# terasum/mythril

Hardware: AMD Instinct MI355X
Metric: constraint-evals/sec (higher is better)
Workload: dtype u32; 1 GPU; synthetic config 5: 10000 random 256-bit constraint tapes x 67108864 assignments per GPU, throughput mode; variant=plain, tapes=10000, rows_per_gpu=67108864, rows_total=67108864, vars=4, mode=count_all, engine=jit, short_circuit=True, parallelism=dp1 (row shards, all-reduce of per-tape results)

## Files before the change

### mythril_amd/csrc/jit.cpp

```cpp
#include "jit.h"

#include <stdarg.h>
#include <stdio.h>
#include <string.h>

#include <algorithm>
#include <atomic>
#include <climits>
#include <cstdlib>
#include <stdexcept>
#include <string>
#include <thread>
#include <unordered_map>
#include <vector>

namespace mh {
namespace jit {

namespace {

struct Fail {
    std::string why;
};

[[noreturn]] void fail(const std::string& w) { throw Fail{w}; }

enum LK : uint8_t { L_UNDEF, L_CONST, L_VGPR };
struct Limb {
    uint8_t k = L_UNDEF;
    uint32_t v = 0;
    static Limb C(uint32_t x) { Limb l; l.k = L_CONST; l.v = x; return l; }
    static Limb R(uint32_t r) { Limb l; l.k = L_VGPR; l.v = r; return l; }
    bool is_c() const { return k == L_CONST; }
    bool is_r() const { return k == L_VGPR; }
    bool is_c(uint32_t x) const { return k == L_CONST && v == x; }
};

struct Val {
    bool is_bool = false;
    int bconst = -1;
    int pair = -1;
    Limb l[8];
    bool defined = false;
};

enum : uint32_t { LBL_SC_SKIP = 0xFFF0, LBL_SC_END = 0xFFF1 };

int top_bit(uint32_t m) { return m ? 31 - __builtin_clz(m) : -1; }
uint32_t prefix_mask(uint32_t m) { int t = top_bit(m); return t < 0 ? 0u : ((2u << t) - 1u); }

class Emitter {
public:
    Emitter(const SsaTape& st, const std::vector<uint32_t>& pool, uint32_t n_vars,
            const Options& opt, const std::vector<uint8_t>* check = nullptr,
            std::vector<double>* insn_cost = nullptr)
        : st_(st), pool_(pool), n_vars_(n_vars), opt_(opt), check_(check),
          insn_cost_(insn_cost) {}

    TapeCode run();

private:
    const SsaTape& st_;
    const std::vector<uint32_t>& pool_;
    uint32_t n_vars_;
    Options opt_;
    const std::vector<uint8_t>* check_;
    std::vector<double>* insn_cost_;
    bool sc_used_ = false;
    std::vector<MI> code_;
    std::vector<Val> vals_;
    std::vector<int> last_;
    std::vector<uint8_t> dem_;
    int vref_[512] = {};
    uint32_t vbase_ = 0, vmax_ = 0, vhigh_ = 0;
    int pref_[N_BOOL_PAIRS] = {};
    uint32_t kstage_ = 0;
    uint32_t n_valu_ = 0, n_wide_ = 0, n_salu_ = 0;
    uint32_t n_valu_cold_ = 0;
    int cold_ = 0;
    bool calls_div_ = false;
    bool uses_lds_ = false;
    bool calls_kec_ = false;
    int cur_op_ = -1;
public:
    static uint64_t op_valu[256], op_wide[256], op_count[256];
// ... 146 lines not shown
    int chain(bool sub, const Limb* a, const Limb* b, int top, Limb* res, uint32_t junk,
              std::vector<uint32_t>& tmp);
    void op_addsub(int d, const Val& A, const Val& B, bool sub);
    void op_logic(int d, const Val& A, const Val& B, int kind);
    Val op_eq(const Val& A, const Val& B);
    void and_all_zero(const std::vector<uint32_t>& regs, int* p, std::vector<uint32_t>& tmp);
    Val op_ult(const Val& A, const Val& B, bool signed_, bool negate);
    void op_ite(int d, const Val& C, const Val& T, const Val& E);
    Val op_bite(const Val& C, const Val& T, const Val& E);
    Val op_bool2(uint8_t op, const Val& A, const Val& B);
    void op_shr(int d, const Val& A, uint32_t s);
    void op_shl(int d, const Val& A, uint32_t s);
    void op_vshift(int d, const Val& A, const Val& B, uint8_t op);
    void op_mul(int d, const Val& A, const Val& B);
    void op_div(int d, int a, int b, int cidx, uint32_t kind, int cur);
    void rescue_div_regs(int cur, uint32_t end = R_TEMP0);
    void op_keccak(const SsaInsn& v, int cur);
    void op_exp(int d, const Val& A, const Val& E);
    void addmod_regs(const uint32_t* u, const uint32_t* v, const uint32_t* n, uint32_t* r,
                     int when = -1);
    void op_mulmod(int d, const Val& X, const Val& Y, const Val& N);
    int scratch_ = -1;
    void demand();
    void sc_check(const Val& v);
    Val& out(int d) {
        Val& v = vals_[d];
        v = Val();
        v.defined = true;
        return v;
    }
};

int Emitter::chain(bool sub, const Limb* a, const Limb* b, int top, Limb* res, uint32_t junk,
                   std::vector<uint32_t>& tmp) {
    int cs = 0;
    uint32_t same = ~0u;
    for (int k = 0; k <= top; ++k) {
        const Limb x = a[k], y = b[k];
        if (x.k == L_UNDEF || y.k == L_UNDEF) fail("internal: chain over an undemanded limb");
        if (cs == 2 && x.is_c() && y.is_c()) {
            const bool through = sub ? x.v == y.v : (uint64_t)x.v + y.v == 0xFFFFFFFFull;
            if (through) {
                if (res) {
                    if (same == ~0u) {
                        same = valloc();
                        emit(M_V_ADDC_CO, {V(same), S(S_DIV_DUMMY, 2), IMM(sub ? 0u : ~0u),
                                           IMM(sub ? 0u : 0u), VCC()}, true);
// ... 76 lines not shown
                    const uint32_t qr = vgpr_of(q, tmp);
                    emit(M_V_ADDC_CO, {V(dst), VCC(), vi_of(p, tmp), V(qr), VCC()});
                }
            } else {
                if (y.is_r()) {
                    emit(M_V_SUBB_CO, {V(dst), VCC(), vi_of(x, tmp), V(y.v), VCC()});
                } else if (x.is_r()) {
                    emit(M_V_SUBBREV_CO, {V(dst), VCC(), vi_of(y, tmp), V(x.v), VCC()});
                } else if (is_inline(x.v) && is_inline(y.v)) {
                    emit(M_V_SUBB_CO, {V(dst), VCC(), IMM(x.v), IMM(y.v), VCC()}, true);
                } else {
                    emit(M_V_SUBB_CO, {V(dst), VCC(), vi_of(x, tmp), V(vgpr_of(y, tmp)), VCC()});
                }
            }
        }
        cs = 2;
        if (res) res[k] = Limb::R(dst);
    }
    return cs;
}

void Emitter::op_addsub(int d, const Val& A, const Val& B, bool sub) {
    const int top = top_bit(dem_[d]);
    Val& R = out(d);
    if (top < 0) return;
    std::vector<uint32_t> tmp;
    chain(sub, A.l, B.l, top, R.l, 0, tmp);
    free_tmp(tmp);
}

void Emitter::op_logic(int d, const Val& A, const Val& B, int kind) {
    const uint32_t dm = dem_[d];
    Val& R = out(d);
    for (int k = 0; k < 8; ++k) {
        if (!((dm >> k) & 1)) continue;
        Limb x = A.l[k], y = B.l[k];
        if (x.is_c() && !y.is_c()) std::swap(x, y);
        if (y.is_c() && ((kind == 0 && y.v == 0) || (kind == 1 && y.v == ~0u))) {
            R.l[k] = Limb::C(y.v);
            continue;
        }
        if (x.k == L_UNDEF || y.k == L_UNDEF) fail("internal: logic over an undemanded limb");
        auto alias = [&](const Limb& l) { R.l[k] = l; if (l.is_r()) vretain(l.v); };
        if (x.is_c() && y.is_c()) {
            R.l[k] = Limb::C(kind == 0 ? (x.v & y.v) : kind == 1 ? (x.v | y.v) : (x.v ^ y.v));
            continue;
// ... 849 lines not shown
                if (l.is_c()) emit(M_V_MOV, {V(dst), IMM(__builtin_bswap32(l.v))});
                else emit(M_V_PERM, {V(dst), IMM(0), V(l.v), S(S_PERM_SEL)});
            }
    free_tmp(tmp);
    for (uint32_t lane = 4 * nw; lane < 25; ++lane)
        for (uint32_t h = 0; h < 2; ++h) {
            uint32_t x = 0;
            if (full && lane == 4 * nw && h == 0) x = 1u;
            if (lane == 16 && h == 1) x = 0x80000000u;
            emit(M_V_MOV, {V(R_KEC0 + 2 * lane + h), IMM(x)});
        }
    emit(M_CALL_KEC, {IMM((uint32_t)code_.size())});
    const KecCode& kc = kec_routine();
    Val& R = out(v.d);
    const uint32_t dm = dem_[v.d];
    for (int k = 0; k < 8; ++k) {
        if (!((dm >> k) & 1)) continue;
        const uint32_t r = valloc();
        emit(M_V_PERM, {V(r), IMM(0), V(kc.out[7 - k]), S(S_PERM_SEL)});
        R.l[k] = Limb::R(r);
    }
}

void Emitter::demand() {
    const auto& code = st_.code;
    const int nv = st_.n_vregs;
    dem_.assign(nv, 0);
    if (st_.root >= 0) dem_[st_.root] = 0xFF;
    auto D = [&](int r, uint32_t m) { if (r >= 0) dem_[r] |= (uint8_t)m; };
    for (size_t i = code.size(); i-- > 0;) {
        const SsaInsn& v = code[i];
        const uint32_t dd = dem_[v.d];
        const uint8_t op = v.op;
        switch (op) {
            case D_NOP: D(v.a, dd); break;
            case D_ADD_R: case D_SUB_R: case D_RSUB_R: case D_MUL_R:
                D(v.a, prefix_mask(dd));
                D(v.b, prefix_mask(dd));
                break;
            case D_AND_R: case D_OR_R: case D_XOR_R: {
                uint32_t ma = dd;
                if (v.cidx >= 0) {
                    for (int k = 0; k < 8; ++k) {
                        const uint32_t c = pool_[8ull * (uint32_t)v.cidx + k];
                        if ((op == D_AND_R && c == 0) || (op == D_OR_R && c == ~0u))
                            ma &= ~(1u << k);
                    }
                }
                D(v.a, ma);
                D(v.b, dd);
                break;
            }
            case D_ITE: D(v.b, dd); D(v.c, dd); break;
            case D_EXP: case D_MULMOD:
                D(v.a, 0xFF);
                D(v.b, 0xFF);
                D(v.c, 0xFF);
                break;
            case D_SHL_V: case D_LSHR_V: case D_ASHR_V:
                D(v.a, 0xFF);
                D(v.b, 0xFF);
                break;
            default:
                if (op >= D_SHR0 && op <= D_SHR7) {
                    const uint32_t s = 32u * (op - D_SHR0) + (v.aux & 31u);
                    const uint32_t q = s >> 5, bsh = s & 31;
                    uint32_t m = 0;
                    for (int k = 0; k < 8; ++k)
                        if ((dd >> k) & 1) {
                            if (k + q < 8) m |= 1u << (k + q);
                            if (bsh && k + q + 1 < 8) m |= 1u << (k + q + 1);
                        }
                    D(v.a, m);
                } else if (op >= D_SHL0 && op <= D_SHL7) {
                    const uint32_t p = op - D_SHL0, f = v.aux & 31u;
                    const uint32_t s = f ? 32u * p + 32u - f : 32u * (p + 1u);
                    if (s < 256) {
                        const int q = (int)(s >> 5), bsh = (int)(s & 31);
                        uint32_t m = 0;
                        for (int k = 0; k < 8; ++k)
                            if ((dd >> k) & 1) {
                                if (k - q >= 0) m |= 1u << (k - q);
                                if (bsh && k - q - 1 >= 0) m |= 1u << (k - q - 1);
                            }
                        D(v.a, m);
                    }
                } else if ((op >= D_EQ_R && op <= D_SGE_C) ||
                           (op >= D_UDIV_R && op <= D_SMOD_C)) {
                    D(v.a, 0xFF);
                    D(v.b, 0xFF);
                } else if (op == D_KECCAK) {
                    D(v.a, 0xFF);
                    D(v.b, 0xFF);
                    D(v.c, 0xFF);
                } else {
                    D(v.a, 0);
                }
                break;
        }
    }
}

uint64_t Emitter::op_valu[256], Emitter::op_wide[256], Emitter::op_count[256];

void Emitter::sc_check(const Val& v) {
    if (!v.is_bool || v.bconst == 1) return;
    sc_used_ = true;
    if (v.bconst == 0) {
        emit(M_S_BRANCH, {LBL(LBL_SC_SKIP)});
        return;
    }
    emit(M_S_AND_B64, {S(S_SCRATCH, 2), P(v.pair), S(S_VALID, 2)});
    emit(M_S_CBRANCH_SCC0, {LBL(LBL_SC_SKIP)});
}

namespace {

double sc_cost(const SsaInsn& v) {
    const uint8_t op = v.op;
    if (op == D_MUL_R) return 60;
    if (op >= D_UDIV_R && op <= D_SMOD_C) return 130;
    if (op == D_SHL_V || op == D_LSHR_V || op == D_ASHR_V) return 35;
    if (op == D_KECCAK) return 7000;
// ... 179 lines not shown
        const int k = order[s];
        for (int i : cone[k])
            if (!done[i]) { out.code.push_back(code[i]); done[i] = 1; }
        if (acc < 0) {
            acc = conj[k];
            check[acc] = 1;
            continue;
        }
        SsaInsn a{};
        a.op = D_BAND;
        a.d = s + 1 == order.size() ? st.root : chain_d[next_d++];
        a.a = acc;
        a.b = conj[k];
        a.c = -1;
        a.width = 1;
        a.cidx = -1;
        out.code.push_back(a);
        acc = a.d;
        if (acc != st.root) check[acc] = 1;
    }
    return true;
}

TapeCode Emitter::run() {
    TapeCode tc;
    tc.alg_ops = st_.alg_ops;
    try {
        const auto& code = st_.code;
        const int nv = st_.n_vregs;
        if (insn_cost_) insn_cost_->assign(code.size(), 0.0);
        const uint32_t n_pin = pinned_cols(n_vars_);
        if (st_.n_pinned != (int)n_pin) fail("assignment columns not pinned as the module pins them");
        bool has_div = false, has_kec = false;
        for (const SsaInsn& v : code) {
            if (v.op == D_KECCAK) { has_kec = true; continue; }
            if (v.op == D_LOADVAR || v.op == D_EXP) continue;
            if (v.op == D_MULMOD && (v.aux & 2u)) continue;
            if (v.op >= D_FIRST_COMPLEX) {
                fail(v.op == D_EXP ? "EXP with a symbolic exponent (interpreter only)"
                     : v.op == D_MULMOD ? "MULMOD (interpreter only)"
                                        : "complex op (interpreter only)");
            }
            if (v.op >= D_UDIV_R && v.op <= D_SMOD_C) has_div = true;
        }
        vbase_ = has_kec ? R_TEMP_KEC : has_div ? R_TEMP0 : n_pin ? R_TEMP_NODIV : R_COL0;
        vmax_ = std::min<uint32_t>(has_kec ? std::max(opt_.max_vgpr, opt_.max_vgpr_keccak)
                                           : opt_.max_vgpr, 256);
        if (vmax_ <= vbase_ + 16) fail("VGPR budget too small");
        vhigh_ = R_COL0 + 8 * n_pin;
        vals_.assign(nv, Val());
        for (int c = 0; c < st_.n_pinned; ++c) {
            Val& v = vals_[c];
            v.defined = true;
            for (int k = 0; k < 8; ++k) v.l[k] = Limb::R(R_COL0 + 8u * (uint32_t)c + k);
        }
        last_.assign(nv, -1);
        for (int i = 0; i < (int)code.size(); ++i)
            for (int r : {code[i].a, code[i].b, code[i].c})
                if (r >= 0) last_[r] = i;
        if (st_.root >= 0) last_[st_.root] = INT_MAX;
        demand();
        scratch_ = nv;
        vals_.push_back(Val());
        last_.push_back(-1);
        dem_.push_back(0xFF);
        for (int i = 0; i < (int)code.size(); ++i) {
            const SsaInsn& v = code[i];
            const uint8_t op = v.op;
            cur_op_ = op;
            const uint32_t valu_before = n_valu_, cold_before = n_valu_cold_;
            ++op_count[op];
            auto Y = [&]() -> Val { return v.cidx >= 0 ? const_val(v.cidx) : val(v.b); };
            switch (op) {
                case D_NOP: {
                    const Val& a = val(v.a);
                    retain(a);
                    vals_[v.d] = a;
                    break;
                }
                case D_LOADC: vals_[v.d] = const_val(v.cidx); break;
                case D_LOADVAR: {
                    const uint32_t dm = dem_[v.d];
                    Val& R = out(v.d);
                    for (int k = 0; k < 8; ++k)
                        if ((dm >> k) & 1u) {
                            const uint32_t r = valloc();
                            emit(M_LOADCOL, {V(r), IMM(8u * v.aux + (uint32_t)k)});
                            R.l[k] = Limb::R(r);
                        }
                    if (dm) emit(M_S_WAITCNT_VM, {IMM(0)});
                    break;
                }
                case D_TRUE: vals_[v.d] = bool_const(true); break;
                case D_FALSE: vals_[v.d] = bool_const(false); break;
                case D_ADD_R: op_addsub(v.d, val(v.a), Y(), false); break;
                case D_SUB_R: op_addsub(v.d, val(v.a), Y(), true); break;
                case D_RSUB_R: op_addsub(v.d, Y(), val(v.a), true); break;
                case D_AND_R: op_logic(v.d, val(v.a), Y(), 0); break;
                case D_OR_R: op_logic(v.d, val(v.a), Y(), 1); break;
                case D_XOR_R: op_logic(v.d, val(v.a), Y(), 2); break;
                case D_EQ_R: vals_[v.d] = op_eq(val(v.a), Y()); break;
                case D_ULT_R: vals_[v.d] = op_ult(val(v.a), Y(), false, false); break;
                case D_UGE_R: vals_[v.d] = op_ult(val(v.a), Y(), false, true); break;
                case D_UGT_R: vals_[v.d] = op_ult(Y(), val(v.a), false, false); break;
                case D_ULE_R: vals_[v.d] = op_ult(Y(), val(v.a), false, true); break;
                case D_SLT_R: vals_[v.d] = op_ult(val(v.a), Y(), true, false); break;
                case D_SGE_R: vals_[v.d] = op_ult(val(v.a), Y(), true, true); break;
                case D_SGT_R: vals_[v.d] = op_ult(Y(), val(v.a), true, false); break;
                case D_SLE_R: vals_[v.d] = op_ult(Y(), val(v.a), true, true); break;
                case D_BAND: case D_BOR: case D_BXOR: case D_BEQ:
                    vals_[v.d] = op_bool2(op, val(v.a), val(v.b));
                    break;
                case D_BNOT: {
                    const Val& a = val(v.a);
                    if (a.bconst >= 0) {
                        vals_[v.d] = bool_const(!a.bconst);
                    } else {
                        const int p = palloc();
                        emit(M_S_NOT_B64, {P(p), P(a.pair)});
                        vals_[v.d] = bool_mask(p);
                    }
                    break;
                }
                case D_ITE: op_ite(v.d, val(v.a), val(v.b), val(v.c)); break;
                case D_BITE: vals_[v.d] = op_bite(val(v.a), val(v.b), val(v.c)); break;
                case D_MUL_R: op_mul(v.d, val(v.a), Y()); break;
                case D_SHL_V: case D_LSHR_V: case D_ASHR_V:
                    op_vshift(v.d, val(v.a), val(v.b), op);
                    break;
                case D_UDIV_R: case D_UREM_R: case D_SDIV_R: case D_SREM_R: case D_SMOD_R:
                    op_div(v.d, v.a, v.b, v.cidx, (uint32_t)(op - D_UDIV_R) >> 1, i);
                    break;
                case D_KECCAK: op_keccak(v, i); break;
                case D_EXP: op_exp(v.d, val(v.a), Y()); break;
                case D_MULMOD: op_mulmod(v.d, val(v.a), val(v.b), val(v.c)); break;
                default:
                    if (op >= D_SHR0 && op <= D_SHR7) {
                        const uint32_t s = 32u * (op - D_SHR0) + (v.aux & 31u);
                        if (s == 0) { const Val& a = val(v.a); retain(a); vals_[v.d] = a; }
                        else op_shr(v.d, val(v.a), s);
                    } else if (op >= D_SHL0 && op <= D_SHL7) {
                        const uint32_t p = op - D_SHL0, f = v.aux & 31u;
                        const uint32_t s = f ? 32u * p + 32u - f : 32u * (p + 1u);
                        if (s >= 256) {
                            Val& R = out(v.d);
                            for (int k = 0; k < 8; ++k) R.l[k] = Limb::C(0);
                        } else {
                            op_shl(v.d, val(v.a), s);
                        }
                    } else {
                        fail("op " + std::to_string(op) + " not in the JIT");
                    }
                    break;
            }
            vals_[v.d].defined = true;
            int seen[3] = {-1, -1, -1};
            int ns = 0;
            for (int r : {v.a, v.b, v.c}) {
                if (r < 0 || last_[r] != i) continue;
                bool dup = false;
                for (int j = 0; j < ns; ++j) dup |= seen[j] == r;
                if (dup) continue;
                seen[ns++] = r;
                release(vals_[r]);
            }
            if (check_ && (*check_)[v.d]) sc_check(vals_[v.d]);
            if (insn_cost_) {
                const bool call = op >= D_UDIV_R && op <= D_SMOD_C;
                (*insn_cost_)[i] = (double)(n_valu_ - valu_before) -
                                   (double)(n_valu_cold_ - cold_before) + (call ? 90.0 : 0.0) +
                                   (op == D_KECCAK ? 7000.0 : 0.0);
            }
        }
        const Val& root = val(st_.root);
        tc.root_bool = root.is_bool;
        if (root.is_bool) {
            if (root.bconst >= 0) emit(M_S_MOV_B64, {S(S_RES, 2), IMM(root.bconst ? ~0u : 0u)});
            else emit(M_S_MOV_B64, {S(S_RES, 2), P(root.pair)});
            if (sc_used_) {
                emit(M_S_BRANCH, {LBL(LBL_SC_END)});
                emit(M_LABEL, {LBL(LBL_SC_SKIP)});
                emit(M_S_MOV_B64, {S(S_RES, 2), IMM(0)});
                emit(M_LABEL, {LBL(LBL_SC_END)});
            }
            for (int k = 0; k < 8; ++k) { tc.root_limbs[k] = ~0u; tc.root_const[k] = 0; }
        } else {
            uint32_t acc = ~0u, cacc = 0;
            for (int k = 0; k < 8; ++k) {
                const Limb l = root.l[k];
                if (l.is_c()) { cacc |= l.v; tc.root_limbs[k] = ~0u; tc.root_const[k] = l.v; continue; }
                tc.root_limbs[k] = l.v;
                tc.root_const[k] = 0;
                if (acc == ~0u) { acc = valloc(); emit(M_V_MOV, {V(acc), V(l.v)}); }
                else emit(M_V_OR, {V(acc), V(l.v), V(acc)});
            }
// ... 1109 lines not shown
    return h;
}

uint32_t default_threads() {
    uint32_t threads = std::max(1u, std::min(4u, std::thread::hardware_concurrency()));
    if (const char* e = std::getenv("MH_JIT_THREADS")) threads = (uint32_t)std::max(1, atoi(e));
    return threads;
}

uint64_t code_id(const std::vector<Built>& built) {
    uint64_t h = 0xcbf29ce484222325ull;
    for (const Built& b : built) {
        h = fnv1a64(&b.text_hash, sizeof b.text_hash, h);
        h = fnv1a64(&b.n_groups, sizeof b.n_groups, h);
    }
    return h;
}

bool build_tapeset(const mh_node* nodes, const uint64_t* offs, uint32_t n_tapes,
                   const uint32_t* consts, uint32_t n_consts, uint32_t n_vars, bool values,
                   const Options& opt, uint32_t threads, std::vector<Built>& out,
                   BuildStats& stats, std::string& err) {
    threads = std::max<uint32_t>(1, std::min<uint32_t>(threads, (n_tapes + 63) / 64));
    out.clear();
    stats.jitted.assign(n_tapes, 0);
    stats.why.assign(n_tapes, std::string());
    struct Slice {
        std::vector<TapeCode> codes;
        std::vector<uint32_t> ids, over;
    };
    std::vector<Slice> slices(threads + 1);
    auto emit_list = [&](const std::vector<uint32_t>& list, const Options& o, Slice& sl,
                         bool keep_over) {
        std::vector<uint32_t> pool;
        ConstIndex index;
        sl.codes.reserve(list.size());
        for (uint32_t t : list) {
            SsaTape st;
            std::string e;
            if (lower_tape_ssa(nodes + offs[t], (size_t)(offs[t + 1] - offs[t]), consts, n_consts,
                               n_vars, pool, index, st, e, true, true) != MH_OK) {
                stats.why[t] = "lowering: " + e;
                continue;
            }
            TapeCode tc = emit_tape(st, pool, n_vars, o);
            if (!tc.ok && !keep_over && pinned_cols(n_vars) == 0 &&
// ... 5 lines not shown
                    tc = emit_tape(st2, pool, n_vars, o);
            }
            if (tc.ok && code_bytes(tc) > 96 * 1024) {
                tc.ok = false;
                tc.why = "tape code larger than 96 KB";
            }
            if (!tc.ok) {
                stats.why[t] = tc.why;
                if (keep_over && tc.why.find("VGPR pressure") != std::string::npos)
                    sl.over.push_back(t);
                continue;
            }
            stats.jitted[t] = 1;
            stats.why[t].clear();
            sl.codes.push_back(std::move(tc));
            sl.ids.push_back(t);
        }
    };
    auto work = [&](uint32_t s) {
        const uint32_t lo = (uint32_t)((uint64_t)n_tapes * s / threads);
        const uint32_t hi = (uint32_t)((uint64_t)n_tapes * (s + 1) / threads);
        std::vector<uint32_t> list;
        for (uint32_t t = lo; t < hi; ++t) list.push_back(t);
        emit_list(list, opt, slices[s], true);
    };
    {
        std::vector<std::thread> pool;
        for (uint32_t s = 1; s < threads; ++s) pool.emplace_back(work, s);
        work(0);
        for (auto& th : pool) th.join();
    }
    std::vector<uint32_t> big;
    for (uint32_t s = 0; s < threads; ++s)
        big.insert(big.end(), slices[s].over.begin(), slices[s].over.end());
    const uint32_t big_budget = std::max(opt.max_vgpr, opt.max_vgpr_keccak);
    if (!big.empty() && big_budget > opt.max_vgpr) {
        Options o2 = opt;
        o2.max_vgpr = big_budget;
        emit_list(big, o2, slices[threads], false);
    }
    const std::vector<uint32_t> cls = occupancy_classes(opt.max_vgpr);
    struct Piece {
        std::vector<const TapeCode*> codes;
        std::vector<uint32_t> ids;
    };
    std::vector<std::vector<std::pair<const TapeCode*, uint32_t>>> bins(cls.size() + 1);
    for (const Slice& sl : slices)
        for (size_t i = 0; i < sl.codes.size(); ++i) {
            const TapeCode& tc = sl.codes[i];
            stats.code_bytes += code_bytes(tc);
            stats.valu_static += tc.n_valu;
            stats.valu_wide_static += tc.n_valu_wide;
            const uint32_t need = module_vgprs(tc, n_vars);
            size_t c = 0;
            while (c < cls.size() && need > cls[c]) ++c;
            bins[c].push_back({&tc, sl.ids[i]});
        }
    const size_t per_piece = std::max<size_t>(64, (n_tapes + threads - 1) / threads);
    std::vector<Piece> pieces;
    for (auto& bin : bins) {
// ... 111 lines not shown
        if (!ok) continue;
        code[q].o[0].v = t;
        for (size_t i = q + 1; i < p; ++i)
            for (int k = 0; k < 5; ++k)
                if (code[i].o[k].k == O_V && code[i].o[k].n == 1 && code[i].o[k].v == x)
                    code[i].o[k].v = t;
        gone[p] = 1;
        ++removed;
    }
    if (removed) {
        std::vector<MI> out;
        out.reserve(code.size() - removed);
        for (size_t i = 0; i < code.size(); ++i)
            if (!gone[i]) out.push_back(code[i]);
        code.swap(out);
    }
    return removed;
}

}

static std::atomic<uint64_t> g_sc_fallbacks{0};

uint64_t sc_fallbacks(bool reset) {
    return reset ? g_sc_fallbacks.exchange(0) : g_sc_fallbacks.load();
}

TapeCode emit_tape(const SsaTape& st, const std::vector<uint32_t>& pool, uint32_t n_vars,
                   const Options& opt) {
    TapeCode tc = emit_tape_body(st, pool, n_vars, opt);
    if (tc.ok && opt.coalesce) {
        const uint32_t r = coalesce_div_moves(tc.code);
        tc.n_valu -= r;
    }
    return tc;
}

TapeCode emit_tape_body(const SsaTape& st, const std::vector<uint32_t>& pool, uint32_t n_vars,
                        const Options& opt) {
    std::vector<double> cost;
    Emitter e(st, pool, n_vars, opt, nullptr, opt.short_circuit ? &cost : nullptr);
    TapeCode tc0 = e.run();
    if (opt.short_circuit) {
        SsaTape sc;
        std::vector<uint8_t> check;
        if (schedule_conjuncts(st, pool, opt.sample_rows, tc0.ok ? &cost : nullptr, sc, check)) {
            Emitter e2(sc, pool, n_vars, opt, &check);
            TapeCode tc = e2.run();
            if (tc.ok) return tc;
            g_sc_fallbacks.fetch_add(1, std::memory_order_relaxed);
        }
    }
    return tc0;
}

}
}
```

### mythril_amd/csrc/jit.h

```cpp
#pragma once
#include <stdint.h>

#include <string>
#include <vector>

#include "compile.h"

namespace mh {
namespace jit {

enum OKind : uint8_t { O_NONE, O_V, O_S, O_VCC, O_IMM, O_LABEL, O_EXEC, O_FONE  };

struct Opnd {
    uint8_t k = O_NONE;
    uint8_t n = 1;
    uint8_t neg = 0;
    uint32_t v = 0;
};

inline Opnd V(uint32_t r, uint8_t n = 1) { Opnd o; o.k = O_V; o.v = r; o.n = n; return o; }
inline Opnd S(uint32_t r, uint8_t n = 1) { Opnd o; o.k = O_S; o.v = r; o.n = n; return o; }
inline Opnd VCC() { Opnd o; o.k = O_VCC; o.n = 2; return o; }
inline Opnd EXEC() { Opnd o; o.k = O_EXEC; o.n = 2; return o; }
inline Opnd IMM(uint32_t x) { Opnd o; o.k = O_IMM; o.v = x; return o; }
// ... 74 lines not shown
};

struct TapeCode {
    bool ok = false;
    std::string why;
    std::vector<MI> code;
    uint32_t max_vgpr = 0;
    bool calls_div = false;
    bool uses_lds = false;
    bool calls_kec = false;
    bool root_bool = true;
    uint32_t root_limbs[8];
    uint32_t root_const[8];
    uint32_t n_valu = 0, n_valu_wide = 0, n_salu = 0;
    uint64_t alg_ops = 0;
};

struct Options {
    uint32_t max_vgpr = 128;
    uint32_t max_vgpr_keccak = 168;
    bool short_circuit = true;
    uint32_t sample_rows = 256;
    bool coalesce = true;
    bool assemble = true;
};

bool schedule_conjuncts(const SsaTape& st, const std::vector<uint32_t>& pool,
                        uint32_t sample_rows, const std::vector<double>* insn_cost, SsaTape& out,
                        std::vector<uint8_t>& check);

TapeCode emit_tape(const SsaTape& st, const std::vector<uint32_t>& pool, uint32_t n_vars,
                   const Options& opt);
TapeCode emit_tape_body(const SsaTape& st, const std::vector<uint32_t>& pool, uint32_t n_vars,
                        const Options& opt);

std::vector<MI> div_routine();

struct KecCode {
    std::vector<MI> code;
    uint32_t out[8];
};
const KecCode& kec_routine();

std::string print(const MI& m, const std::string& prefix);
void print_list(const std::vector<MI>& code, const std::string& prefix, std::string& out);

// ... 61 lines not shown
```

Before: 410.0 billion evals/s.

## Add staged cheap pre-filter of short-circuit conjunct compares in JIT emitter

Reorders each short-circuit conjunct so the instructions feeding its compare form a slice. That slice is first evaluated on a single 32-bit limb (limb 0 for equality, the top limb with carry-slack bounds for ordered compares), so lanes that cannot satisfy the conjunct are masked off before the full 256-bit evaluation. The goal is to avoid wide multi-limb arithmetic for rows that a cheap partial check already rejects. The cost is extra emitted compares, extra emitter passes and a re-emit when a stage is rejected, and added correctness risk in the slack reasoning. It is on by default at level 3, controlled by MH_JIT_STAGE.

```diff
diff --git a/mythril_amd/csrc/jit.cpp b/mythril_amd/csrc/jit.cpp
--- a/mythril_amd/csrc/jit.cpp
+++ b/mythril_amd/csrc/jit.cpp
@@ -46,6 +46,8 @@
 
 enum : uint32_t { LBL_SC_SKIP = 0xFFF0, LBL_SC_END = 0xFFF1 };
 
+constexpr uint32_t kStageMargin = 8;
+
 int top_bit(uint32_t m) { return m ? 31 - __builtin_clz(m) : -1; }
 uint32_t prefix_mask(uint32_t m) { int t = top_bit(m); return t < 0 ? 0u : ((2u << t) - 1u); }
 
@@ -60,7 +62,7 @@
     TapeCode run();
 
 private:
-    const SsaTape& st_;
+    SsaTape st_;
     const std::vector<uint32_t>& pool_;
     uint32_t n_vars_;
     Options opt_;
@@ -253,7 +255,24 @@
     void op_mulmod(int d, const Val& X, const Val& Y, const Val& N);
     int scratch_ = -1;
     void demand();
+    template <class F> void demand_rule(const SsaInsn& v, uint32_t dd, F&& D);
     void sc_check(const Val& v);
+    void emit_insn(int i, bool slice, bool no_check);
+    struct Stage { int first_e, ic, acc; };
+    struct Slack { uint32_t lo = 0, hi = 0; };
+public:
+    int stage_ = 0;
+    const std::vector<uint8_t>* stage_skip_ = nullptr;
+    std::vector<int> stage_rejected_;
+private:
+    std::vector<Stage> stages_;
+    std::vector<Slack> slack_;
+    std::vector<uint8_t> slack_ok_;
+    bool in_slice_ = false;
+    void plan_stages();
+    void emit_staged(const Stage& sg);
+    void cmp32(uint16_t op, Limb x, Limb y);
+    bool stage_decide(const SsaInsn& c, int q, int acc);
     Val& out(int d) {
         Val& v = vals_[d];
         v = Val();
@@ -376,6 +395,25 @@
 
 void Emitter::op_addsub(int d, const Val& A, const Val& B, bool sub) {
     const int top = top_bit(dem_[d]);
+    if (in_slice_ && slack_ok_[d]) {
+        const Limb x = A.l[7], y = B.l[7];
+        if (x.k == L_UNDEF || y.k == L_UNDEF) fail("internal: slice over an undemanded top limb");
+        Val& R = out(d);
+        if (x.is_c() && y.is_c()) {
+            R.l[7] = Limb::C(sub ? x.v - y.v : x.v + y.v);
+        } else {
+            const uint32_t dst = valloc();
+            if (!sub) {
+                if (y.is_r()) emit(M_V_ADD_U32, {V(dst), src(x), V(y.v)});
+                else emit(M_V_ADD_U32, {V(dst), src(y), V(x.v)});
+            } else {
+                if (y.is_r()) emit(M_V_SUB_U32, {V(dst), src(x), V(y.v)});
+                else emit(M_V_SUBREV_U32, {V(dst), src(y), V(x.v)});
+            }
+            R.l[7] = Limb::R(dst);
+        }
+        return;
+    }
     Val& R = out(d);
     if (top < 0) return;
     std::vector<uint32_t> tmp;
@@ -1271,83 +1309,84 @@
     }
 }
 
+template <class F>
+void Emitter::demand_rule(const SsaInsn& v, uint32_t dd, F&& D) {
+    const uint8_t op = v.op;
+    switch (op) {
+        case D_NOP: D(v.a, dd); break;
+        case D_ADD_R: case D_SUB_R: case D_RSUB_R: case D_MUL_R:
+            D(v.a, prefix_mask(dd));
+            D(v.b, prefix_mask(dd));
+            break;
+        case D_AND_R: case D_OR_R: case D_XOR_R: {
+            uint32_t ma = dd;
+            if (v.cidx >= 0) {
+                for (int k = 0; k < 8; ++k) {
+                    const uint32_t c = pool_[8ull * (uint32_t)v.cidx + k];
+                    if ((op == D_AND_R && c == 0) || (op == D_OR_R && c == ~0u))
+                        ma &= ~(1u << k);
+                }
+            }
+            D(v.a, ma);
+            D(v.b, dd);
+            break;
+        }
+        case D_ITE: D(v.b, dd); D(v.c, dd); break;
+        case D_EXP: case D_MULMOD:
+            D(v.a, 0xFF);
+            D(v.b, 0xFF);
+            D(v.c, 0xFF);
+            break;
+        case D_SHL_V: case D_LSHR_V: case D_ASHR_V:
+            D(v.a, 0xFF);
+            D(v.b, 0xFF);
+            break;
+        default:
+            if (op >= D_SHR0 && op <= D_SHR7) {
+                const uint32_t s = 32u * (op - D_SHR0) + (v.aux & 31u);
+                const uint32_t q = s >> 5, bsh = s & 31;
+                uint32_t m = 0;
+                for (int k = 0; k < 8; ++k)
+                    if ((dd >> k) & 1) {
+                        if (k + q < 8) m |= 1u << (k + q);
+                        if (bsh && k + q + 1 < 8) m |= 1u << (k + q + 1);
+                    }
+                D(v.a, m);
+            } else if (op >= D_SHL0 && op <= D_SHL7) {
+                const uint32_t p = op - D_SHL0, f = v.aux & 31u;
+                const uint32_t s = f ? 32u * p + 32u - f : 32u * (p + 1u);
+                if (s < 256) {
+                    const int q = (int)(s >> 5), bsh = (int)(s & 31);
+                    uint32_t m = 0;
+                    for (int k = 0; k < 8; ++k)
+                        if ((dd >> k) & 1) {
+                            if (k - q >= 0) m |= 1u << (k - q);
+                            if (bsh && k - q - 1 >= 0) m |= 1u << (k - q - 1);
+                        }
+                    D(v.a, m);
+                }
+            } else if ((op >= D_EQ_R && op <= D_SGE_C) ||
+                       (op >= D_UDIV_R && op <= D_SMOD_C)) {
+                D(v.a, 0xFF);
+                D(v.b, 0xFF);
+            } else if (op == D_KECCAK) {
+                D(v.a, 0xFF);
+                D(v.b, 0xFF);
+                D(v.c, 0xFF);
+            } else {
+                D(v.a, 0);
+            }
+            break;
+    }
+}
+
 void Emitter::demand() {
     const auto& code = st_.code;
     const int nv = st_.n_vregs;
     dem_.assign(nv, 0);
     if (st_.root >= 0) dem_[st_.root] = 0xFF;
     auto D = [&](int r, uint32_t m) { if (r >= 0) dem_[r] |= (uint8_t)m; };
-    for (size_t i = code.size(); i-- > 0;) {
-        const SsaInsn& v = code[i];
-        const uint32_t dd = dem_[v.d];
-        const uint8_t op = v.op;
-        switch (op) {
-            case D_NOP: D(v.a, dd); break;
-            case D_ADD_R: case D_SUB_R: case D_RSUB_R: case D_MUL_R:
-                D(v.a, prefix_mask(dd));
-                D(v.b, prefix_mask(dd));
-                break;
-            case D_AND_R: case D_OR_R: case D_XOR_R: {
-                uint32_t ma = dd;
-                if (v.cidx >= 0) {
-                    for (int k = 0; k < 8; ++k) {
-                        const uint32_t c = pool_[8ull * (uint32_t)v.cidx + k];
-                        if ((op == D_AND_R && c == 0) || (op == D_OR_R && c == ~0u))
-                            ma &= ~(1u << k);
-                    }
-                }
-                D(v.a, ma);
-                D(v.b, dd);
-                break;
-            }
-            case D_ITE: D(v.b, dd); D(v.c, dd); break;
-            case D_EXP: case D_MULMOD:
-                D(v.a, 0xFF);
-                D(v.b, 0xFF);
-                D(v.c, 0xFF);
-                break;
-            case D_SHL_V: case D_LSHR_V: case D_ASHR_V:
-                D(v.a, 0xFF);
-                D(v.b, 0xFF);
-                break;
-            default:
-                if (op >= D_SHR0 && op <= D_SHR7) {
-                    const uint32_t s = 32u * (op - D_SHR0) + (v.aux & 31u);
-                    const uint32_t q = s >> 5, bsh = s & 31;
-                    uint32_t m = 0;
-                    for (int k = 0; k < 8; ++k)
-                        if ((dd >> k) & 1) {
-                            if (k + q < 8) m |= 1u << (k + q);
-                            if (bsh && k + q + 1 < 8) m |= 1u << (k + q + 1);
-                        }
-                    D(v.a, m);
-                } else if (op >= D_SHL0 && op <= D_SHL7) {
-                    const uint32_t p = op - D_SHL0, f = v.aux & 31u;
-                    const uint32_t s = f ? 32u * p + 32u - f : 32u * (p + 1u);
-                    if (s < 256) {
-                        const int q = (int)(s >> 5), bsh = (int)(s & 31);
-                        uint32_t m = 0;
-                        for (int k = 0; k < 8; ++k)
-                            if ((dd >> k) & 1) {
-                                if (k - q >= 0) m |= 1u << (k - q);
-                                if (bsh && k - q - 1 >= 0) m |= 1u << (k - q - 1);
-                            }
-                        D(v.a, m);
-                    }
-                } else if ((op >= D_EQ_R && op <= D_SGE_C) ||
-                           (op >= D_UDIV_R && op <= D_SMOD_C)) {
-                    D(v.a, 0xFF);
-                    D(v.b, 0xFF);
-                } else if (op == D_KECCAK) {
-                    D(v.a, 0xFF);
-                    D(v.b, 0xFF);
-                    D(v.c, 0xFF);
-                } else {
-                    D(v.a, 0);
-                }
-                break;
-        }
-    }
+    for (size_t i = code.size(); i-- > 0;) demand_rule(code[i], dem_[code[i].d], D);
 }
 
 uint64_t Emitter::op_valu[256], Emitter::op_wide[256], Emitter::op_count[256];
@@ -1573,10 +1612,379 @@
     return true;
 }
 
+namespace {
+bool is_compare(uint8_t op) { return op >= D_EQ_R && op <= D_SGE_C; }
+bool sliceable(uint8_t op) {
+    return op == D_NOP || op == D_LOADC || op == D_ADD_R || op == D_SUB_R || op == D_RSUB_R ||
+           op == D_AND_R || op == D_OR_R || op == D_XOR_R || op == D_ITE || op == D_MUL_R ||
+           (op >= D_SHR0 && op <= D_SHL7) || is_compare(op) || (op >= D_BAND && op <= D_FALSE) ||
+           op == D_BITE;
+}
+}
+
+void Emitter::plan_stages() {
+    const std::vector<SsaInsn> code = st_.code;
+    const int n = (int)code.size(), nv = st_.n_vregs;
+    std::vector<std::vector<int>> users(nv);
+    for (int i = 0; i < n; ++i)
+        for (int r : {code[i].a, code[i].b, code[i].c})
+            if (r >= 0 && r < nv) users[r].push_back(i);
+    std::vector<SsaInsn> out;
+    out.reserve(code.size());
+    std::vector<char> excl(n, 0);
+    bool seen_first = false;
+    int start = 0;
+    for (int i = 0; i < n; ++i) {
+        const SsaInsn& v = code[i];
+        if (v.d < 0 || v.d >= nv) return;
+        const bool first = !seen_first && (*check_)[v.d];
+        const bool band = seen_first && v.op == D_BAND && ((*check_)[v.d] || v.d == st_.root);
+        if (!first && !band) continue;
+        seen_first = true;
+        const int ic = first ? i : i - 1;
+        bool cand = ic >= start && is_compare(code[ic].op) && users[code[ic].d].size() == 1 &&
+                    (first || code[ic].d == v.b) && code[ic].d != st_.root &&
+                    !(stage_skip_ && (*stage_skip_)[code[ic].d]);
+        if (cand && code[ic].op != D_EQ_R && stage_ < 2) cand = false;
+        bool any = false;
+        if (cand) {
+            for (int j = ic - 1; j >= start; --j) {
+                const int d = code[j].d;
+                bool ok = sliceable(code[j].op) && d != st_.root && d >= st_.n_pinned;
+                for (int u : users[d]) ok = ok && (u == ic || (u >= start && u < ic && excl[u]));
+                excl[j] = ok;
+                any |= ok;
+            }
+        }
+        if (cand && any) {
+            for (int j = start; j < ic; ++j)
+                if (!excl[j]) out.push_back(code[j]);
+            Stage sg;
+            sg.first_e = (int)out.size();
+            for (int j = start; j < ic; ++j)
+                if (excl[j]) out.push_back(code[j]);
+            sg.ic = (int)out.size();
+            sg.acc = first ? -1 : v.a;
+            out.push_back(code[ic]);
+            stages_.push_back(sg);
+        } else {
+            for (int j = start; j <= ic; ++j) out.push_back(code[j]);
+        }
+        if (!first) out.push_back(code[i]);
+        start = i + 1;
+    }
+    for (int j = start; j < n; ++j) out.push_back(code[j]);
+    st_.code.swap(out);
+}
+
+void Emitter::cmp32(uint16_t op, Limb x, Limb y) {
+    if (y.is_c() && !x.is_c()) {
+        const uint16_t rev = op == M_V_CMP_LT ? M_V_CMP_GT
+                           : op == M_V_CMP_LT_I32 ? M_V_CMP_GT_I32 : op;
+        emit(rev, {VCC(), IMM(y.v), V(x.v)});
+    } else {
+        emit(op, {VCC(), src(x), V(y.v)});
+    }
+}
+
+bool Emitter::stage_decide(const SsaInsn& c, int q, int acc) {
+    const Val A0 = val(c.a);
+    const Val B0 = c.cidx >= 0 ? const_val(c.cidx) : val(c.b);
+    auto live = [&](Opnd und) {
+        if (acc >= 0 && val(acc).bconst < 0) {
+            emit(M_S_AND_B64, {P(q), und, P(val(acc).pair)});
+            emit(M_S_AND_B64, {P(q), P(q), S(S_VALID, 2)});
+        } else {
+            emit(M_S_AND_B64, {P(q), und, S(S_VALID, 2)});
+        }
+    };
+    if (c.op == D_EQ_R) {
+        Limb x = A0.l[0], y = B0.l[0];
+        if (x.k == L_UNDEF || y.k == L_UNDEF) return false;
+        if (x.is_c() && y.is_c()) return false;
+        if (x.is_r() && y.is_r() && x.v == y.v) return false;
+        if (!y.is_r()) std::swap(x, y);
+        emit(M_V_CMP_EQ, {VCC(), src(x), V(y.v)});
+        live(VCC());
+        return true;
+    }
+    const uint8_t k = (uint8_t)((c.op - D_ULT_R) >> 1);
+    const bool swap = (k & 3) == 1 || (k & 3) == 2, signed_ = k >= 4;
+    const Val& A = swap ? B0 : A0;
+    const Val& B = swap ? A0 : B0;
+    const int ra = swap ? (c.cidx >= 0 ? -1 : c.b) : c.a, rb = swap ? c.a : (c.cidx >= 0 ? -1 : c.b);
+    const Limb x = A.l[7], y = B.l[7];
+    if (x.k == L_UNDEF || y.k == L_UNDEF) return false;
+    if (x.is_c() && y.is_c()) return false;
+    if (x.is_r() && y.is_r() && x.v == y.v) return false;
+    const Slack sx = ra >= 0 ? slack_[ra] : Slack(), sy = rb >= 0 ? slack_[rb] : Slack();
+    const uint32_t D = sx.lo + sx.hi + sy.lo + sy.hi;
+    const uint32_t bias = signed_ ? 0x80000000u : 0u;
+    std::vector<uint32_t> tmp;
+    if (D == 0) {
+        cmp32(M_V_CMP_EQ, x, y);
+        live(VCC());
+    } else {
+        if (D > 64) return false;
+        for (int s = 0; s < 2; ++s) {
+            const Limb l = s ? y : x;
+            const Slack sl = s ? sy : sx;
+            if (!l.is_c()) continue;
+            const uint32_t v = l.v ^ bias;
+            if (v < sl.lo || v > 0xFFFFFFFFu - sl.hi) return false;
+        }
+        const uint32_t e = valloc();
+        tmp.push_back(e);
+        if (y.is_c()) {
+            emit(M_V_ADD_U32, {V(e), IMM(D - y.v), V(x.v)});
+        } else if (x.is_c()) {
+            emit(M_V_SUB_U32, {V(e), IMM(x.v + D), V(y.v)});
+        } else {
+            emit(M_V_SUB_U32, {V(e), V(x.v), V(y.v)});
+            emit(M_V_ADD_U32, {V(e), IMM(D), V(e)});
+        }
+        emit(M_V_CMP_GT, {VCC(), IMM(2 * D + 1), V(e)});
+        bool in_q = false;
+        for (int s = 0; s < 2; ++s) {
+            const Limb l = s ? y : x;
+            const Slack sl = s ? sy : sx;
+            if (l.is_c() || sl.lo + sl.hi == 0) continue;
+            if (!in_q) { emit(M_S_MOV_B64, {P(q), VCC()}); in_q = true; }
+            emit(M_V_ADD_U32, {V(e), IMM(bias - sl.lo), V(l.v)});
+            emit(M_V_CMP_LT, {VCC(), IMM(0xFFFFFFFFu - sl.hi - sl.lo), V(e)});
+            emit(M_S_OR_B64, {P(q), P(q), VCC()});
+        }
+        live(in_q ? P(q) : VCC());
+    }
+    free_tmp(tmp);
+    return true;
+}
+
+void Emitter::emit_staged(const Stage& sg) {
+    const SsaInsn& c = st_.code[sg.ic];
+    const int nv = st_.n_vregs;
+    const bool eq = c.op == D_EQ_R;
+    const int q = palloc();
+    std::vector<uint8_t> sd(nv, 0), exact(nv, 0);
+    auto ask = [&](int r, uint32_t m, bool ex) {
+        if (r < 0 || r >= nv) return;
+        sd[r] |= (uint8_t)m;
+        if (ex && m) exact[r] = 1;
+    };
+    const bool open_carry = stage_ >= 3 && !eq;
+    ask(c.a, eq ? 0x01u : 0x80u, !open_carry);
+    if (c.cidx < 0) ask(c.b, eq ? 0x01u : 0x80u, !open_carry);
+    slack_ok_.assign(nv, 0);
+    for (int j = sg.ic - 1; j >= sg.first_e; --j) {
+        const SsaInsn& v = st_.code[j];
+        const uint32_t dd = sd[v.d];
+        const bool ex = exact[v.d] != 0;
+        if (open_carry && !ex && dd == 0x80u &&
+            (v.op == D_ADD_R || v.op == D_SUB_R || v.op == D_RSUB_R)) {
+            slack_ok_[v.d] = 1;
+            ask(v.a, 0x80u, false);
+            if (v.cidx < 0) ask(v.b, 0x80u, false);
+        } else if (v.op == D_NOP) {
+            ask(v.a, dd, ex);
+        } else if (v.op == D_ITE) {
+            ask(v.b, dd, ex);
+            ask(v.c, dd, ex);
+        } else {
+            demand_rule(v, dd, [&](int r, uint32_t m) { ask(r, m, true); });
+        }
+    }
+    const uint32_t hot0 = n_valu_ - n_valu_cold_;
+    std::vector<uint8_t> saved(sg.ic - sg.first_e);
+    slack_.assign(nv, Slack());
+    in_slice_ = true;
+    for (int j = sg.first_e; j < sg.ic; ++j) {
+        const SsaInsn& v = st_.code[j];
+        saved[j - sg.first_e] = dem_[v.d];
+        dem_[v.d] = sd[v.d];
+        const bool is_val = !(is_compare(v.op) || (v.op >= D_BAND && v.op <= D_FALSE) ||
+                              v.op == D_BITE);
+        if (is_val && sd[v.d] == 0) {
+            out(v.d);
+            continue;
+        }
+        emit_insn(j, true, true);
+        const Slack a = v.a >= 0 ? slack_[v.a] : Slack();
+        const Slack b = v.cidx < 0 && v.b >= 0 ? slack_[v.b] : Slack();
+        Slack r;
+        if (slack_ok_[v.d]) {
+            if (v.op == D_ADD_R) { r.lo = a.lo + b.lo; r.hi = a.hi + b.hi + 1; }
+            else if (v.op == D_SUB_R) { r.lo = a.lo + b.hi + 1; r.hi = a.hi + b.lo; }
+            else { r.lo = b.lo + a.hi + 1; r.hi = b.hi + a.lo; }
+        } else if (v.op == D_NOP) {
+            r = a;
+        } else if (v.op == D_ITE) {
+            const Slack t = slack_[v.b], e = slack_[v.c];
+            r.lo = std::max(t.lo, e.lo);
+            r.hi = std::max(t.hi, e.hi);
+        }
+        slack_[v.d] = r;
+    }
+    in_slice_ = false;
+    cur_op_ = c.op;
+    const bool decided = stage_decide(c, q, sg.acc);
+    uint32_t l_cold = 0, l_join = 0;
+    if (decided) {
+        l_join = next_lbl_++;
+        if (eq) {
+            emit(M_S_CBRANCH_SCC0, {LBL(l_join)});
+        } else {
+            l_cold = next_lbl_++;
+            emit(M_S_CBRANCH_SCC1, {LBL(l_cold)});
+            const uint8_t k = (uint8_t)((c.op - D_ULT_R) >> 1);
+            const bool swap = (k & 3) == 1 || (k & 3) == 2, negate = (k & 3) >= 2, signed_ = k >= 4;
+            const Val A0 = val(c.a);
+            const Val B0 = c.cidx >= 0 ? const_val(c.cidx) : val(c.b);
+            const Limb x = (swap ? B0 : A0).l[7], y = (swap ? A0 : B0).l[7];
+            cmp32(signed_ ? M_V_CMP_LT_I32 : M_V_CMP_LT, x, y);
+            emit(negate ? M_S_NOT_B64 : M_S_MOV_B64, {P(q), VCC()});
+            emit(M_S_BRANCH, {LBL(l_join)});
+            emit(M_LABEL, {LBL(l_cold)});
+        }
+    }
+    const uint32_t hot = (n_valu_ - n_valu_cold_) - hot0;
+    for (int j = sg.first_e; j < sg.ic; ++j) {
+        const SsaInsn& v = st_.code[j];
+        if (vals_[v.d].defined) release(vals_[v.d]);
+        vals_[v.d] = Val();
+        dem_[v.d] = saved[j - sg.first_e];
+    }
+    const uint32_t full0 = n_valu_ - n_valu_cold_;
+    for (int j = sg.first_e; j <= sg.ic; ++j) emit_insn(j, false, true);
+    const uint32_t full = (n_valu_ - n_valu_cold_) - full0;
+    n_valu_cold_ += full;
+    const Val r = vals_[c.d];
+    cur_op_ = c.op;
+    if (r.bconst >= 0) {
+        emit(M_S_MOV_B64, {P(q), IMM(r.bconst ? 0xFFFFFFFFu : 0u)});
+    } else {
+        emit(M_S_MOV_B64, {P(q), P(r.pair)});
+        release(r);
+    }
+    if (decided) emit(M_LABEL, {LBL(l_join)});
+    vals_[c.d] = bool_mask(q);
+    if (!decided || hot + kStageMargin > full) stage_rejected_.push_back(c.d);
+    if (check_ && (*check_)[c.d]) sc_check(vals_[c.d]);
+}
+
+void Emitter::emit_insn(int i, bool slice, bool no_check) {
+    const SsaInsn& v = st_.code[i];
+    const uint8_t op = v.op;
+    cur_op_ = op;
+    const uint32_t valu_before = n_valu_, cold_before = n_valu_cold_;
+    ++op_count[op];
+    auto Y = [&]() -> Val { return v.cidx >= 0 ? const_val(v.cidx) : val(v.b); };
+    switch (op) {
+        case D_NOP: {
+            const Val& a = val(v.a);
+            retain(a);
+            vals_[v.d] = a;
+            break;
+        }
+        case D_LOADC: vals_[v.d] = const_val(v.cidx); break;
+        case D_LOADVAR: {
+            const uint32_t dm = dem_[v.d];
+            Val& R = out(v.d);
+            for (int k = 0; k < 8; ++k)
+                if ((dm >> k) & 1u) {
+                    const uint32_t r = valloc();
+                    emit(M_LOADCOL, {V(r), IMM(8u * v.aux + (uint32_t)k)});
+                    R.l[k] = Limb::R(r);
+                }
+            if (dm) emit(M_S_WAITCNT_VM, {IMM(0)});
+            break;
+        }
+        case D_TRUE: vals_[v.d] = bool_const(true); break;
+        case D_FALSE: vals_[v.d] = bool_const(false); break;
+        case D_ADD_R: op_addsub(v.d, val(v.a), Y(), false); break;
+        case D_SUB_R: op_addsub(v.d, val(v.a), Y(), true); break;
+        case D_RSUB_R: op_addsub(v.d, Y(), val(v.a), true); break;
+        case D_AND_R: op_logic(v.d, val(v.a), Y(), 0); break;
+        case D_OR_R: op_logic(v.d, val(v.a), Y(), 1); break;
+        case D_XOR_R: op_logic(v.d, val(v.a), Y(), 2); break;
+        case D_EQ_R: vals_[v.d] = op_eq(val(v.a), Y()); break;
+        case D_ULT_R: vals_[v.d] = op_ult(val(v.a), Y(), false, false); break;
+        case D_UGE_R: vals_[v.d] = op_ult(val(v.a), Y(), false, true); break;
+        case D_UGT_R: vals_[v.d] = op_ult(Y(), val(v.a), false, false); break;
+        case D_ULE_R: vals_[v.d] = op_ult(Y(), val(v.a), false, true); break;
+        case D_SLT_R: vals_[v.d] = op_ult(val(v.a), Y(), true, false); break;
+        case D_SGE_R: vals_[v.d] = op_ult(val(v.a), Y(), true, true); break;
+        case D_SGT_R: vals_[v.d] = op_ult(Y(), val(v.a), true, false); break;
+        case D_SLE_R: vals_[v.d] = op_ult(Y(), val(v.a), true, true); break;
+        case D_BAND: case D_BOR: case D_BXOR: case D_BEQ:
+            vals_[v.d] = op_bool2(op, val(v.a), val(v.b));
+            break;
+        case D_BNOT: {
+            const Val& a = val(v.a);
+            if (a.bconst >= 0) {
+                vals_[v.d] = bool_const(!a.bconst);
+            } else {
+                const int p = palloc();
+                emit(M_S_NOT_B64, {P(p), P(a.pair)});
+                vals_[v.d] = bool_mask(p);
+            }
+            break;
+        }
+        case D_ITE: op_ite(v.d, val(v.a), val(v.b), val(v.c)); break;
+        case D_BITE: vals_[v.d] = op_bite(val(v.a), val(v.b), val(v.c)); break;
+        case D_MUL_R: op_mul(v.d, val(v.a), Y()); break;
+        case D_SHL_V: case D_LSHR_V: case D_ASHR_V:
+            op_vshift(v.d, val(v.a), val(v.b), op);
+            break;
+        case D_UDIV_R: case D_UREM_R: case D_SDIV_R: case D_SREM_R: case D_SMOD_R:
+            op_div(v.d, v.a, v.b, v.cidx, (uint32_t)(op - D_UDIV_R) >> 1, i);
+            break;
+        case D_KECCAK: op_keccak(v, i); break;
+        case D_EXP: op_exp(v.d, val(v.a), Y()); break;
+        case D_MULMOD: op_mulmod(v.d, val(v.a), val(v.b), val(v.c)); break;
+        default:
+            if (op >= D_SHR0 && op <= D_SHR7) {
+                const uint32_t s = 32u * (op - D_SHR0) + (v.aux & 31u);
+                if (s == 0) { const Val& a = val(v.a); retain(a); vals_[v.d] = a; }
+                else op_shr(v.d, val(v.a), s);
+            } else if (op >= D_SHL0 && op <= D_SHL7) {
+                const uint32_t p = op - D_SHL0, f = v.aux & 31u;
+                const uint32_t s = f ? 32u * p + 32u - f : 32u * (p + 1u);
+                if (s >= 256) {
+                    Val& R = out(v.d);
+                    for (int k = 0; k < 8; ++k) R.l[k] = Limb::C(0);
+                } else {
+                    op_shl(v.d, val(v.a), s);
+                }
+            } else {
+                fail("op " + std::to_string(op) + " not in the JIT");
+            }
+            break;
+    }
+    vals_[v.d].defined = true;
+    int seen[3] = {-1, -1, -1};
+    int ns = 0;
+    for (int r : {v.a, v.b, v.c}) {
+        if (slice || r < 0 || last_[r] != i) continue;
+        bool dup = false;
+        for (int j = 0; j < ns; ++j) dup |= seen[j] == r;
+        if (dup) continue;
+        seen[ns++] = r;
+        release(vals_[r]);
+    }
+    if (check_ && !slice && !no_check && (*check_)[v.d]) sc_check(vals_[v.d]);
+    if (insn_cost_ && !slice) {
+        const bool call = op >= D_UDIV_R && op <= D_SMOD_C;
+        (*insn_cost_)[i] = (double)(n_valu_ - valu_before) -
+                           (double)(n_valu_cold_ - cold_before) + (call ? 90.0 : 0.0) +
+                           (op == D_KECCAK ? 7000.0 : 0.0);
+    }
+}
+
 TapeCode Emitter::run() {
     TapeCode tc;
     tc.alg_ops = st_.alg_ops;
     try {
+        if (check_ && stage_ > 0) plan_stages();
         const auto& code = st_.code;
         const int nv = st_.n_vregs;
         if (insn_cost_) insn_cost_->assign(code.size(), 0.0);
@@ -1615,113 +2023,14 @@
         vals_.push_back(Val());
         last_.push_back(-1);
         dem_.push_back(0xFF);
+        size_t si = 0;
         for (int i = 0; i < (int)code.size(); ++i) {
-            const SsaInsn& v = code[i];
-            const uint8_t op = v.op;
-            cur_op_ = op;
-            const uint32_t valu_before = n_valu_, cold_before = n_valu_cold_;
-            ++op_count[op];
-            auto Y = [&]() -> Val { return v.cidx >= 0 ? const_val(v.cidx) : val(v.b); };
-            switch (op) {
-                case D_NOP: {
-                    const Val& a = val(v.a);
-                    retain(a);
-                    vals_[v.d] = a;
-                    break;
-                }
-                case D_LOADC: vals_[v.d] = const_val(v.cidx); break;
-                case D_LOADVAR: {
-                    const uint32_t dm = dem_[v.d];
-                    Val& R = out(v.d);
-                    for (int k = 0; k < 8; ++k)
-                        if ((dm >> k) & 1u) {
-                            const uint32_t r = valloc();
-                            emit(M_LOADCOL, {V(r), IMM(8u * v.aux + (uint32_t)k)});
-                            R.l[k] = Limb::R(r);
-                        }
-                    if (dm) emit(M_S_WAITCNT_VM, {IMM(0)});
-                    break;
-                }
-                case D_TRUE: vals_[v.d] = bool_const(true); break;
-                case D_FALSE: vals_[v.d] = bool_const(false); break;
-                case D_ADD_R: op_addsub(v.d, val(v.a), Y(), false); break;
-                case D_SUB_R: op_addsub(v.d, val(v.a), Y(), true); break;
-                case D_RSUB_R: op_addsub(v.d, Y(), val(v.a), true); break;
-                case D_AND_R: op_logic(v.d, val(v.a), Y(), 0); break;
-                case D_OR_R: op_logic(v.d, val(v.a), Y(), 1); break;
-                case D_XOR_R: op_logic(v.d, val(v.a), Y(), 2); break;
-                case D_EQ_R: vals_[v.d] = op_eq(val(v.a), Y()); break;
-                case D_ULT_R: vals_[v.d] = op_ult(val(v.a), Y(), false, false); break;
-                case D_UGE_R: vals_[v.d] = op_ult(val(v.a), Y(), false, true); break;
-                case D_UGT_R: vals_[v.d] = op_ult(Y(), val(v.a), false, false); break;
-                case D_ULE_R: vals_[v.d] = op_ult(Y(), val(v.a), false, true); break;
-                case D_SLT_R: vals_[v.d] = op_ult(val(v.a), Y(), true, false); break;
-                case D_SGE_R: vals_[v.d] = op_ult(val(v.a), Y(), true, true); break;
-                case D_SGT_R: vals_[v.d] = op_ult(Y(), val(v.a), true, false); break;
-                case D_SLE_R: vals_[v.d] = op_ult(Y(), val(v.a), true, true); break;
-                case D_BAND: case D_BOR: case D_BXOR: case D_BEQ:
-                    vals_[v.d] = op_bool2(op, val(v.a), val(v.b));
-                    break;
-                case D_BNOT: {
-                    const Val& a = val(v.a);
-                    if (a.bconst >= 0) {
-                        vals_[v.d] = bool_const(!a.bconst);
-                    } else {
-                        const int p = palloc();
-                        emit(M_S_NOT_B64, {P(p), P(a.pair)});
-                        vals_[v.d] = bool_mask(p);
-                    }
-                    break;
-                }
-                case D_ITE: op_ite(v.d, val(v.a), val(v.b), val(v.c)); break;
-                case D_BITE: vals_[v.d] = op_bite(val(v.a), val(v.b), val(v.c)); break;
-                case D_MUL_R: op_mul(v.d, val(v.a), Y()); break;
-                case D_SHL_V: case D_LSHR_V: case D_ASHR_V:
-                    op_vshift(v.d, val(v.a), val(v.b), op);
-                    break;
-                case D_UDIV_R: case D_UREM_R: case D_SDIV_R: case D_SREM_R: case D_SMOD_R:
-                    op_div(v.d, v.a, v.b, v.cidx, (uint32_t)(op - D_UDIV_R) >> 1, i);
-                    break;
-                case D_KECCAK: op_keccak(v, i); break;
-                case D_EXP: op_exp(v.d, val(v.a), Y()); break;
-                case D_MULMOD: op_mulmod(v.d, val(v.a), val(v.b), val(v.c)); break;
-                default:
-                    if (op >= D_SHR0 && op <= D_SHR7) {
-                        const uint32_t s = 32u * (op - D_SHR0) + (v.aux & 31u);
-                        if (s == 0) { const Val& a = val(v.a); retain(a); vals_[v.d] = a; }
-                        else op_shr(v.d, val(v.a), s);
-                    } else if (op >= D_SHL0 && op <= D_SHL7) {
-                        const uint32_t p = op - D_SHL0, f = v.aux & 31u;
-                        const uint32_t s = f ? 32u * p + 32u - f : 32u * (p + 1u);
-                        if (s >= 256) {
-                            Val& R = out(v.d);
-                            for (int k = 0; k < 8; ++k) R.l[k] = Limb::C(0);
-                        } else {
-                            op_shl(v.d, val(v.a), s);
-                        }
-                    } else {
-                        fail("op " + std::to_string(op) + " not in the JIT");
-                    }
-                    break;
-            }
-            vals_[v.d].defined = true;
-            int seen[3] = {-1, -1, -1};
-            int ns = 0;
-            for (int r : {v.a, v.b, v.c}) {
-                if (r < 0 || last_[r] != i) continue;
-                bool dup = false;
-                for (int j = 0; j < ns; ++j) dup |= seen[j] == r;
-                if (dup) continue;
-                seen[ns++] = r;
-                release(vals_[r]);
-            }
-            if (check_ && (*check_)[v.d]) sc_check(vals_[v.d]);
-            if (insn_cost_) {
-                const bool call = op >= D_UDIV_R && op <= D_SMOD_C;
-                (*insn_cost_)[i] = (double)(n_valu_ - valu_before) -
-                                   (double)(n_valu_cold_ - cold_before) + (call ? 90.0 : 0.0) +
-                                   (op == D_KECCAK ? 7000.0 : 0.0);
-            }
+            if (si < stages_.size() && stages_[si].first_e == i) {
+                emit_staged(stages_[si]);
+                i = stages_[si++].ic;
+                continue;
+            }
+            emit_insn(i, false, false);
         }
         const Val& root = val(st_.root);
         tc.root_bool = root.is_bool;
@@ -2877,6 +3186,8 @@
                    const Options& opt, uint32_t threads, std::vector<Built>& out,
                    BuildStats& stats, std::string& err) {
     threads = std::max<uint32_t>(1, std::min<uint32_t>(threads, (n_tapes + 63) / 64));
+    Options eopt = opt;
+    if (values) eopt.stage = 0;
     out.clear();
     stats.jitted.assign(n_tapes, 0);
     stats.why.assign(n_tapes, std::string());
@@ -2928,7 +3239,7 @@
         const uint32_t hi = (uint32_t)((uint64_t)n_tapes * (s + 1) / threads);
         std::vector<uint32_t> list;
         for (uint32_t t = lo; t < hi; ++t) list.push_back(t);
-        emit_list(list, opt, slices[s], true);
+        emit_list(list, eopt, slices[s], true);
     };
     {
         std::vector<std::thread> pool;
@@ -2941,7 +3252,7 @@
         big.insert(big.end(), slices[s].over.begin(), slices[s].over.end());
     const uint32_t big_budget = std::max(opt.max_vgpr, opt.max_vgpr_keccak);
     if (!big.empty() && big_budget > opt.max_vgpr) {
-        Options o2 = opt;
+        Options o2 = eopt;
         o2.max_vgpr = big_budget;
         emit_list(big, o2, slices[threads], false);
     }
@@ -3099,6 +3410,11 @@
 
 static std::atomic<uint64_t> g_sc_fallbacks{0};
 
+static int stage_level() {
+    const char* e = std::getenv("MH_JIT_STAGE");
+    return e ? std::min(3, std::max(0, atoi(e))) : 3;
+}
+
 uint64_t sc_fallbacks(bool reset) {
     return reset ? g_sc_fallbacks.exchange(0) : g_sc_fallbacks.load();
 }
@@ -3122,6 +3438,21 @@
         SsaTape sc;
         std::vector<uint8_t> check;
         if (schedule_conjuncts(st, pool, opt.sample_rows, tc0.ok ? &cost : nullptr, sc, check)) {
+            const int level = opt.stage >= 0 ? opt.stage : stage_level();
+            if (level > 0) {
+                Emitter e2(sc, pool, n_vars, opt, &check);
+                e2.stage_ = level;
+                TapeCode tc = e2.run();
+                if (tc.ok && !e2.stage_rejected_.empty()) {
+                    std::vector<uint8_t> skip((size_t)sc.n_vregs, 0);
+                    for (int d : e2.stage_rejected_) skip[(size_t)d] = 1;
+                    Emitter e3(sc, pool, n_vars, opt, &check);
+                    e3.stage_ = level;
+                    e3.stage_skip_ = &skip;
+                    tc = e3.run();
+                }
+                if (tc.ok) return tc;
+            }
             Emitter e2(sc, pool, n_vars, opt, &check);
             TapeCode tc = e2.run();
             if (tc.ok) return tc;
diff --git a/mythril_amd/csrc/jit.h b/mythril_amd/csrc/jit.h
--- a/mythril_amd/csrc/jit.h
+++ b/mythril_amd/csrc/jit.h
@@ -120,6 +120,7 @@
     bool short_circuit = true;
     uint32_t sample_rows = 256;
     bool coalesce = true;
+    int stage = -1;
     bool assemble = true;
 };
 
```

Result: faster. 431.3 billion evals/s, median of 6 (+5.2%).
